# muzishen/RCDMs

Measured on AMD Instinct MI355X. Metric: story-frames/sec (stage-2 UNet, 50-step DDIM, 512^2), higher is better.
Workload: dtype f16; 1 GPU; PororoSV stage-2, 512x512, 50-step DDIM, CFG 2.0, batch=1 story x 5 frames per GPU, ctx 85x768, random-init 1276.9M-param UNet3D; stories_per_gpu=1, latent=64, ddim_steps=50, parallelism=story-replicas x1

## Files before the change

rcdms_amd/csrc/igemm16.hip:

```cpp
#include "common.h"
#include "igemm_args.h"
#include "pp_sync.h"
#include "igemm_epilogue.h"
#ifndef RCDM_I16_ABLATE
#define RCDM_I16_ABLATE 0
#endif

namespace {

template <int TAPS, bool SLAB>
__global__ __launch_bounds__(256, 2) void igemm16_kernel(const IgemmArgs p) {
  constexpr int BM = 160, BN = 160, FM = 5, FN = 5;
  constexpr int A_BYTES = BM * 128, STAGE = (BM + BN) * 128;
  constexpr int NP = BM / 8 / 4;
  extern __shared__ __attribute__((aligned(16))) char smem[];

  const int t = threadIdx.x, lane = t & 63;
  const int wave = __builtin_amdgcn_readfirstlane(t >> 6);
  const int wm = wave >> 1, wn = wave & 1;
  const int ks_begin = blockIdx.y * p.nk_per_split;
  const int nkl = min(p.nk, ks_begin + p.nk_per_split) - ks_begin;
  if (nkl <= 0) return;

  int cm0, cn0;
  {
    const int ntiles = p.tilesM * p.tilesN, lin = blockIdx.x;
    const int xcd = lin & 7, q = ntiles >> 3, r = ntiles & 7;
    const int tl = (xcd < r ? xcd * (q + 1) : r * (q + 1) + (xcd - r) * q) + (lin >> 3);
    constexpr int GM = 8;
    const int per_group = GM * p.tilesN;
    const int sg = tl / per_group, rem = tl - sg * per_group;
    const int gm = min(GM, p.tilesM - sg * GM);
    const int tn = rem / gm, tm = sg * GM + (rem - tn * gm);
    cm0 = tm * BM;
    cn0 = tn * BN;
  }

  f32x2 lx_pre = {1.f, 0.f};
  const bool lx_on = TAPS == 1 && !SLAB && p.lnx_stat != nullptr;
  LnxRow<1, kLnxMaxParts> lx_row0;
  if (lx_on && t < BM) lx_row0.load(p.lnx_stat, p.lnx_ld, cm0 + t, cm0 + t < p.M, p.lnx_parts, 0);

  const __amdgpu_buffer_rsrc_t rsrcA = __builtin_amdgcn_make_buffer_rsrc((void*)p.A, 0, 0x7FFFFFFF, 0x00020000);
  const __amdgpu_buffer_rsrc_t rsrcW = __builtin_amdgcn_make_buffer_rsrc((void*)p.W, 0, 0x7FFFFFFF, 0x00020000);
  const __amdgpu_buffer_rsrc_t rsrcA2 = __builtin_amdgcn_make_buffer_rsrc((void*)(TAPS == 9 ? p.A2 : p.A), 0, 0x7FFFFFFF, 0x00020000);
  constexpr unsigned OOB = 0x80000000u;
  const int Hv = p.Hi << p.up, Wv = p.Wi << p.up;
  const int lrow = lane >> 3, lch = lane & 7;

  unsigned a_off[NP], w_off[NP];
  int a_img[NP], a_iy[NP], a_ix[NP], a_c[NP], w_c[NP];
#pragma unroll
  for (int i = 0; i < NP; ++i) {
    const int row = (wave * NP + i) * 8 + lrow;
    const int m = cm0 + row;
    a_c[i] = (lch ^ ((row >> 1) & 7)) * 8;
    a_off[i] = OOB;
    a_img[i] = a_ix[i] = 0;
    a_iy[i] = -(1 << 20);
    if (TAPS == 1) {
      if (m < p.M) a_off[i] = (unsigned)m * (unsigned)p.lda * 2u;
    } else if (m < p.M) {
      const int hw = p.Ho * p.Wo;
      const int img = m / hw, rem = m - img * hw;
      const int oy = rem / p.Wo, ox = rem - oy * p.Wo;
      a_img[i] = img * p.Hi * p.Wi;
      a_iy[i] = oy * p.stride - p.pad;
      a_ix[i] = ox * p.stride - p.pad;
    }
    const int n = cn0 + row;
    w_c[i] = a_c[i];
    w_off[i] = n < p.N ? (unsigned)n * (unsigned)p.Ktot * 2u : OOB;
  }
  auto issue = [&](int g, int stage) __attribute__((always_inline)) {
    const int ks = ks_begin + g;
    int tap = 0, kci = ks;
    const bool s2 = TAPS == 9 && ks >= p.nk1;
    if (TAPS != 1) {
      kci = ks / 9;
      tap = ks - kci * 9;
      if (s2) {
        kci = ks - p.nk1;
        tap = 9;
      }
    }
    const int c0 = kci * BK;
    const int dy = s2 ? 1 : tap / 3, dx = s2 ? 1 : tap - dy * 3;
    const int cin = s2 ? p.Cin2 : p.Cin;
    const unsigned lda = (unsigned)(s2 ? p.lda2 : p.lda);
    char* sbase = smem + stage * STAGE;
#pragma unroll
    for (int i = 0; i < NP; ++i) {
      const int c = c0 + a_c[i];
      unsigned vo;
      if (TAPS == 1) {
        vo = (c < p.Cin && a_off[i] != OOB) ? a_off[i] + (unsigned)c * 2u : OOB;
      } else {
        const int iy = a_iy[i] + dy, ix = a_ix[i] + dx;
        const bool ok = (c < cin) && ((unsigned)iy < (unsigned)Hv) && ((unsigned)ix < (unsigned)Wv);
        const int sy = iy >> p.up, sx = ix >> p.up;
        const unsigned off = ((unsigned)(a_img[i] + sy * p.Wi + sx) * lda + (unsigned)c) * 2u;
        vo = ok ? off : OOB;
      }
      if (TAPS == 9 && s2)
        __builtin_amdgcn_raw_ptr_buffer_load_lds(
            rsrcA2, (__attribute__((address_space(3))) void*)(sbase + (wave * NP + i) * 1024), 16, vo, 0, 0, 0);
      else
        __builtin_amdgcn_raw_ptr_buffer_load_lds(
            rsrcA, (__attribute__((address_space(3))) void*)(sbase + (wave * NP + i) * 1024), 16, vo, 0, 0, 0);
    }
#if RCDM_I16_ABLATE & 16
    if (g > 0) return;
#endif
#pragma unroll
    for (int i = 0; i < NP; ++i) {
      const int c = c0 + w_c[i];
      const unsigned vo = (c < cin && w_off[i] != OOB)
                              ? w_off[i] + ((unsigned)tap * (unsigned)p.Cin + (unsigned)c) * 2u : OOB;
      __builtin_amdgcn_raw_ptr_buffer_load_lds(
          rsrcW, (__attribute__((address_space(3))) void*)(sbase + A_BYTES + (wave * NP + i) * 1024), 16, vo, 0, 0, 0);
    }
  };

  const int l15 = lane & 15, kg = lane >> 4;
  const int sw = (lane >> 1) & 7;
  const int koff0 = ((kg ^ sw) << 4), koff1 = (((4 + kg) ^ sw) << 4);
  const int rowA = (wm * (BM / 2) + l15) * 128, rowB = A_BYTES + (wn * (BN / 2) + l15) * 128;
  f32x4 acc[FN][FM];
#pragma unroll
  for (int i = 0; i < FN; ++i)
#pragma unroll
    for (int j = 0; j < FM; ++j) acc[i][j] = f32x4{0.f, 0.f, 0.f, 0.f};

  constexpr int kStg = BM * (2 * BN + 16);
  static_assert(lnx_table_bytes(BM, BN) <= 4096 && 4096 + kStg <= 2 * STAGE && kStg >= STAGE, "epilogue layout");
  const bool lx_low = lx_on && !(nkl & 1);
  float* const lx_tab = (float*)(smem + (lx_low ? 0 : kStg));
  char* const stg = smem + (lx_low ? 4096 : 0);
  issue(0, 0);
  if (lx_on && t < BM) {
    float r_ = 1.f, m_ = 0.f;
    lx_row0.finish(p.lnx_invC, p.lnx_eps, r_, m_);
    lx_pre = f32x2{r_, m_};
  }
  for (int g = 0; g < nkl; ++g) {
    wait_vm<0>();
    __builtin_amdgcn_s_barrier();
#if !(RCDM_I16_ABLATE & 8)
    if (g + 1 < nkl) issue(g + 1, (g + 1) & 1);
#endif
    const char* sb = smem + (g & 1) * STAGE;
#if RCDM_PRIO_LOADS
    __builtin_amdgcn_s_setprio(3);
#endif
#pragma unroll
    for (int kk = 0; kk < 2; ++kk) {
      const int koff = kk ? koff1 : koff0;
      f16x8 wf[FN], xf[FM];
#pragma unroll
      for (int i = 0; i < FN; ++i) wf[i] = *(const f16x8*)(sb + rowB + i * 2048 + koff);
#pragma unroll
      for (int j = 0; j < FM; ++j) xf[j] = *(const f16x8*)(sb + rowA + j * 2048 + koff);
#if RCDM_PRIO_LOADS
      __builtin_amdgcn_s_setprio(0);
#endif
#pragma unroll
      for (int i = 0; i < FN; ++i)
#pragma unroll
        for (int j = 0; j < FM; ++j) acc[i][j] = __builtin_amdgcn_mfma_f32_16x16x32_f16(wf[i], xf[j], acc[i][j], 0, 0, 0);
#if RCDM_PRIO_LOADS
      __builtin_amdgcn_s_setprio(3);
#endif
    }
  }
  if constexpr (TAPS == 1 && !SLAB)
    if (lx_on) lnx_write_tables<BM, BN>(p, lx_tab, cm0, cn0, t, lx_pre);
  wait_lgkm0();
  tick_barrier();
#if RCDM_I16_ABLATE & 1
  {
    float s = 0.f;
#pragma unroll
    for (int i = 0; i < FN; ++i)
#pragma unroll
      for (int j = 0; j < FM; ++j) s += acc[i][j][0] + acc[i][j][1] + acc[i][j][2] + acc[i][j][3];
    if (s == 1.2345678e33f) p.out[0] = (f16)s;
  }
#else
  if constexpr (SLAB) {
    if (p.slab16) {
      IgemmArgs q{};
      q.out = (f16*)p.partial + (size_t)blockIdx.y * p.M * p.N;
      q.M = p.M; q.N = p.N; q.ldc = p.N; q.epi = 0; q.out_scale = 1.0f; q.dup = 0;
      tile_epilogue<FM, FN, false, 256, BM, BN, false, false>(q, smem, acc, cm0, cn0, wm * (BM / 2), wn * (BN / 2), l15, kg, t, nullptr);
      return;
    }
  }
  tile_epilogue<FM, FN, SLAB, 256, BM, BN, false, TAPS == 1 && !SLAB>(p, stg, acc, cm0, cn0, wm * (BM / 2), wn * (BN / 2), l15, kg, t,
                                                                       lx_on ? lx_tab : nullptr);
#endif
}

constexpr int kLds16 = 2 * (160 + 160) * 128;

template <int TAPS>
int launch16(const IgemmArgs& a, hipStream_t stream) {
  static bool attr_set[64] = {};
  if (rcdm_first_on_device(attr_set)) {
    (void)hipFuncSetAttribute((const void*)igemm16_kernel<TAPS, false>, hipFuncAttributeMaxDynamicSharedMemorySize, kLds16);
    (void)hipFuncSetAttribute((const void*)igemm16_kernel<TAPS, true>, hipFuncAttributeMaxDynamicSharedMemorySize, kLds16);
  }
  dim3 grid(a.tilesM * a.tilesN, a.splits);
  if (a.splits > 1)
    hipLaunchKernelGGL((igemm16_kernel<TAPS, true>), grid, dim3(256), kLds16, stream, a);
  else
    hipLaunchKernelGGL((igemm16_kernel<TAPS, false>), grid, dim3(256), kLds16, stream, a);
  return rcdm_check_launch();
}

}

int rcdm_igemm16_launch(const IgemmArgs& a, int taps, hipStream_t stream) {
  if (taps == 1) return launch16<1>(a, stream);
  if (taps == 9) return launch16<9>(a, stream);
  return RCDM_EINVAL;
}
```

rcdms_amd/csrc/wino.hip:

```cpp
#include "common.h"
#include "igemm_args.h"
#include "pp_sync.h"
#include "igemm_epilogue.h"
#include <stdlib.h>

namespace {

struct WinoArgs {
  const f16* in;
  const f16* in2;
  const f16* U;
  const f16* W2;
  const float* bias;
  const float* rowvec;
  const f16* res;
  f16* out;
  f16* V;
  float* slab;
  int slab16;
  int n_img, H, W, th, tw, T, N, K, K2;
  int lda, lda2, ldc, ldr, ldt, rows_per_sample;
  int epi;
  float out_scale;
  int E, splits, nk, nk2, nkps, nkps2, tilesM, tilesN;
  const float* gn_stat;
  const float* gn_gamma;
  const float* gn_beta;
  int gn_cg, gn_G, gn_rps, gn_silu;
  float* go_partial;
  int go_G, go_cg, go_rps, go_splits;
};

__global__ __launch_bounds__(256) void wino_in_kernel(const WinoArgs p) {
  const int nch = p.K >> 2;
  const int idx = blockIdx.x * 256 + threadIdx.x;
  if (idx >= p.T * nch) return;
  const int t = idx / nch, c4 = idx - t * nch;
  const int tpi = p.th * p.tw;
  const int img = t / tpi, rem = t - img * tpi;
  const int ty = rem / p.tw, tx = rem - ty * p.tw;
  typedef unsigned u32x2_t __attribute__((ext_vector_type(2)));
  union H4 { u32x2_t v; f16 e[4]; f16x4 h; };
  const __amdgpu_buffer_rsrc_t rs = __builtin_amdgcn_make_buffer_rsrc((void*)p.in, 0, 0x7FFFFFFF, 0x00020000);
  const unsigned base = ((unsigned)(img * p.H * p.W) * (unsigned)p.lda + (unsigned)c4 * 4u) * 2u;
  H4 d[4][4];
  bool ok[4][4];
#pragma unroll
  for (int i = 0; i < 4; ++i)
#pragma unroll
    for (int j = 0; j < 4; ++j) {
      const int y = 2 * ty - 1 + i, x = 2 * tx - 1 + j;
      ok[i][j] = (unsigned)y < (unsigned)p.H && (unsigned)x < (unsigned)p.W;
      const unsigned off = ok[i][j] ? base + (unsigned)(y * p.W + x) * (unsigned)p.lda * 2u : 0x80000000u;
      d[i][j].v = __builtin_amdgcn_raw_buffer_load_b64(rs, off, 0, 0);
    }
  f32x4 sc = {1.f, 1.f, 1.f, 1.f}, sh = {0.f, 0.f, 0.f, 0.f};
  const bool gn = p.gn_stat != nullptr;
  if (gn) {
    const int s = (img * p.H * p.W) / p.gn_rps;
    const f32x4 ga = *(const f32x4*)(p.gn_gamma + c4 * 4), be = *(const f32x4*)(p.gn_beta + c4 * 4);
#pragma unroll
    for (int e = 0; e < 4; ++e) {
      const int g = (c4 * 4 + e) / p.gn_cg;
      const f32x2 mr = *(const f32x2*)(p.gn_stat + (size_t)(s * p.gn_G + g) * 2);
      sc[e] = mr.y * ga[e];
      sh[e] = __builtin_fmaf(-(mr.x * mr.y), ga[e], be[e]);
    }
  }
  float f[4][4][4];
#pragma unroll
  for (int i = 0; i < 4; ++i)
#pragma unroll
    for (int j = 0; j < 4; ++j)
#pragma unroll
      for (int e = 0; e < 4; ++e) {
        float v = (float)d[i][j].e[e];
        if (gn) {
          v = __builtin_fmaf(v, sc[e], sh[e]);
          if (p.gn_silu) v = silu_f(v);
          if (!ok[i][j]) v = 0.f;
        }
        f[i][j][e] = v;
      }
  float r[4][4][4];
#pragma unroll
  for (int j = 0; j < 4; ++j)
#pragma unroll
    for (int e = 0; e < 4; ++e) {
      r[0][j][e] = f[0][j][e] - f[2][j][e];
      r[1][j][e] = f[1][j][e] + f[2][j][e];
      r[2][j][e] = f[2][j][e] - f[1][j][e];
      r[3][j][e] = f[1][j][e] - f[3][j][e];
    }
  f16* vb = p.V + (size_t)t * p.K + c4 * 4;
  const size_t pstride = (size_t)p.T * p.K;
#pragma unroll
  for (int i = 0; i < 4; ++i) {
    H4 o[4];
#pragma unroll
    for (int e = 0; e < 4; ++e) {
      o[0].e[e] = (f16)(r[i][0][e] - r[i][2][e]);
      o[1].e[e] = (f16)(r[i][1][e] + r[i][2][e]);
      o[2].e[e] = (f16)(r[i][2][e] - r[i][1][e]);
      o[3].e[e] = (f16)(r[i][1][e] - r[i][3][e]);
    }
#pragma unroll
    for (int j = 0; j < 4; ++j) *(u32x2_t*)(vb + (size_t)(i * 4 + j) * pstride) = o[j].v;
  }
}

template <bool S16>
__global__ __launch_bounds__(256, 2) void wino_gemm_kernel(const WinoArgs p) {
  constexpr int BM = 160, BN = 160, FM = 5, FN = 5;
  constexpr int A_BYTES = BM * 128, STAGE = (BM + BN) * 128;
  constexpr int NP = BM / 8 / 4;
  extern __shared__ __attribute__((aligned(16))) char smem[];

  const int t = threadIdx.x, lane = t & 63;
  const int wave = __builtin_amdgcn_readfirstlane(t >> 6);
  const int wm = wave >> 1, wn = wave & 1;
  const int ntile = p.tilesM * p.tilesN, W = p.E * p.splits * ntile;
  const int n_extra = p.E - 16;
  int item;
  {
    const int lin = blockIdx.x, xcd = lin & 7, j = lin >> 3;
    const int WX = n_extra * p.splits * ntile, WM = W - WX;
    if (((WX | WM) & 7) == 0) {
      const int xq = WX >> 3, mq = WM >> 3;
      item = j < xq ? xcd * xq + j : WX + xcd * mq + (j - xq);
    } else {
      const int q = W >> 3, r = W & 7;
      item = (xcd < r ? xcd * (q + 1) : r * (q + 1) + (xcd - r) * q) + j;
    }
  }
  const int yes = item / ntile, tl = item - yes * ntile;
  const int ye = yes / p.splits, split = yes - ye * p.splits;
  const int entry = ye < n_extra ? 16 + ye : ye - n_extra;
  const bool extra = entry >= 16;
  const int nk = extra ? p.nk2 : p.nk, nkps = extra ? p.nkps2 : p.nkps;
  const int ks_begin = split * nkps;
  const int nkl = min(nk, ks_begin + nkps) - ks_begin;
  const int Kd = extra ? p.K2 : p.K;
  const size_t slab_off = ((size_t)entry * p.splits + split) * p.T * p.N;

  const int tn = tl / p.tilesM, tm = tl - tn * p.tilesM;
  const int cm0 = tm * BM, cn0 = tn * BN;
  const f16* Abase = extra ? p.in2 : p.V + (size_t)entry * p.T * p.K;
  const f16* Wbase = extra ? p.W2 : p.U + (size_t)entry * p.N * p.K;
  const __amdgpu_buffer_rsrc_t rsrcA = __builtin_amdgcn_make_buffer_rsrc((void*)Abase, 0, 0x7FFFFFFF, 0x00020000);
  const __amdgpu_buffer_rsrc_t rsrcW = __builtin_amdgcn_make_buffer_rsrc((void*)Wbase, 0, 0x7FFFFFFF, 0x00020000);
  constexpr unsigned OOB = 0x80000000u;
  const int lrow = lane >> 3, lch = lane & 7;

  unsigned a_off[NP], w_off[NP];
  int a_c[NP];
#pragma unroll
  for (int i = 0; i < NP; ++i) {
    const int row = (wave * NP + i) * 8 + lrow;
    const int m = cm0 + row;
    a_c[i] = (lch ^ ((row >> 1) & 7)) * 8;
    a_off[i] = OOB;
    if (m < p.T) {
      if (extra) {
        const int tpi = p.th * p.tw;
        const int img = m / tpi, rem = m - img * tpi;
        const int ty = rem / p.tw, tx = rem - ty * p.tw;
        const int ab = entry - 16;
        const int prow = img * p.H * p.W + (2 * ty + (ab >> 1)) * p.W + 2 * tx + (ab & 1);
        a_off[i] = (unsigned)prow * (unsigned)p.lda2 * 2u;
      } else {
        a_off[i] = (unsigned)m * (unsigned)p.K * 2u;
      }
    }
    const int n = cn0 + row;
    w_off[i] = n < p.N ? (unsigned)n * (unsigned)Kd * 2u : OOB;
  }
  auto issue = [&](int g, int stage) __attribute__((always_inline)) {
    const int c0 = (ks_begin + g) * BK;
    char* sbase = smem + stage * STAGE;
#pragma unroll
    for (int i = 0; i < NP; ++i) {
      const int c = c0 + a_c[i];
      const unsigned vo = (c < Kd && a_off[i] != OOB) ? a_off[i] + (unsigned)c * 2u : OOB;
      __builtin_amdgcn_raw_ptr_buffer_load_lds(
          rsrcA, (__attribute__((address_space(3))) void*)(sbase + (wave * NP + i) * 1024), 16, vo, 0, 0, 0);
    }
#pragma unroll
    for (int i = 0; i < NP; ++i) {
      const int c = c0 + a_c[i];
      const unsigned vo = (c < Kd && w_off[i] != OOB) ? w_off[i] + (unsigned)c * 2u : OOB;
      __builtin_amdgcn_raw_ptr_buffer_load_lds(
          rsrcW, (__attribute__((address_space(3))) void*)(sbase + A_BYTES + (wave * NP + i) * 1024), 16, vo, 0, 0, 0);
    }
  };

  const int l15 = lane & 15, kg = lane >> 4;
  const int sw = (lane >> 1) & 7;
  const int koff0 = ((kg ^ sw) << 4), koff1 = (((4 + kg) ^ sw) << 4);
  const int rowA = (wm * (BM / 2) + l15) * 128, rowB = A_BYTES + (wn * (BN / 2) + l15) * 128;
  f32x4 acc[FN][FM];
#pragma unroll
  for (int i = 0; i < FN; ++i)
#pragma unroll
    for (int j = 0; j < FM; ++j) acc[i][j] = f32x4{0.f, 0.f, 0.f, 0.f};

  if (nkl > 0) issue(0, 0);
  for (int g = 0; g < nkl; ++g) {
    wait_vm<0>();
    __builtin_amdgcn_s_barrier();
    if (g + 1 < nkl) issue(g + 1, (g + 1) & 1);
    const char* sb = smem + (g & 1) * STAGE;
    __builtin_amdgcn_s_setprio(3);
#pragma unroll
    for (int kk = 0; kk < 2; ++kk) {
      const int koff = kk ? koff1 : koff0;
      f16x8 wf[FN], xf[FM];
#pragma unroll
      for (int i = 0; i < FN; ++i) wf[i] = *(const f16x8*)(sb + rowB + i * 2048 + koff);
#pragma unroll
      for (int j = 0; j < FM; ++j) xf[j] = *(const f16x8*)(sb + rowA + j * 2048 + koff);
      __builtin_amdgcn_s_setprio(0);
#pragma unroll
      for (int i = 0; i < FN; ++i)
#pragma unroll
        for (int j = 0; j < FM; ++j) acc[i][j] = __builtin_amdgcn_mfma_f32_16x16x32_f16(wf[i], xf[j], acc[i][j], 0, 0, 0);
      __builtin_amdgcn_s_setprio(3);
    }
  }
  const int row0 = wm * (BM / 2), col0 = wn * (BN / 2);
  if constexpr (S16) {
    wait_lgkm0();
    tick_barrier();
    IgemmArgs q{};
    q.out = (f16*)p.slab + slab_off;
    q.M = p.T; q.N = p.N; q.ldc = p.N; q.epi = 0; q.out_scale = 1.0f; q.dup = 0;
    tile_epilogue<FM, FN, false, 256, BM, BN, false, false>(q, smem, acc, cm0, cn0, row0, col0, l15, kg, t, nullptr);
  } else {
    wait_lgkm0();
    tick_barrier();
    slab_store_staged<FM, FN, 256, BM, BN, 80>(p.slab + slab_off, p.N, p.T, p.N, smem, acc, cm0, cn0, row0, col0, l15, kg, t);
  }
}

template <bool S16>
__device__ __forceinline__ f32x4 slab_load4(const WinoArgs& p, size_t off) {
  if constexpr (S16) {
    union { uint2 u; f16 e[4]; } h;
    h.u = *(const uint2*)((const f16*)p.slab + off);
    return f32x4{(float)h.e[0], (float)h.e[1], (float)h.e[2], (float)h.e[3]};
  } else {
    return *(const f32x4*)(p.slab + off);
  }
}

template <int SP, bool S16>
__global__ __launch_bounds__(512) void wino_out_kernel(const WinoArgs p) {
  extern __shared__ __attribute__((aligned(16))) char smem[];
  const int nch = p.N >> 2;
  const int t = blockIdx.x;
  const int tpi = p.th * p.tw;
  const int img = t / tpi, rem = t - img * tpi;
  const int ty = rem / p.tw, tx = rem - ty * p.tw;
  const size_t splane = (size_t)p.T * p.N, eplane = (size_t)p.splits * splane;
  int prow[4];
#pragma unroll
  for (int ab = 0; ab < 4; ++ab) prow[ab] = img * p.H * p.W + (2 * ty + (ab >> 1)) * p.W + 2 * tx + (ab & 1);
  union H4 { uint2 u; f16 e[4]; };
  for (int cg4 = threadIdx.x; cg4 < nch; cg4 += blockDim.x) {
    const int n = cg4 * 4;
    const size_t src = (size_t)t * p.N + n;
    H4 rr[4];
#pragma unroll
    for (int ab = 0; ab < 4; ++ab) {
      rr[ab].u = make_uint2(0, 0);
      if (p.epi & RCDM_EPI_RESIDUAL) rr[ab].u = *(const uint2*)(p.res + (size_t)prow[ab] * p.ldr + n);
    }
    f32x4 m[16];
#pragma unroll
    for (int e = 0; e < 16; ++e) m[e] = slab_load4<S16>(p, src + e * eplane);
    if constexpr (SP == 2) {
      f32x4 m2[16];
#pragma unroll
      for (int e = 0; e < 16; ++e) m2[e] = slab_load4<S16>(p, src + e * eplane + splane);
#pragma unroll
      for (int e = 0; e < 16; ++e) m[e] += m2[e];
    } else if constexpr (SP == 0) {
      for (int s = 1; s < p.splits; ++s) {
        f32x4 m2[16];
#pragma unroll
        for (int e = 0; e < 16; ++e) m2[e] = slab_load4<S16>(p, src + e * eplane + s * splane);
#pragma unroll
        for (int e = 0; e < 16; ++e) m[e] += m2[e];
      }
    }
    f32x4 o[4];
    {
      f32x4 r0[4], r1[4];
#pragma unroll
      for (int j = 0; j < 4; ++j) {
        r0[j] = m[0 * 4 + j] + m[1 * 4 + j] + m[2 * 4 + j];
        r1[j] = m[1 * 4 + j] - m[2 * 4 + j] - m[3 * 4 + j];
      }
      o[0] = r0[0] + r0[1] + r0[2];
      o[1] = r0[1] - r0[2] - r0[3];
      o[2] = r1[0] + r1[1] + r1[2];
      o[3] = r1[1] - r1[2] - r1[3];
    }
    if (p.E > 16) {
      f32x4 x[4];
#pragma unroll
      for (int ab = 0; ab < 4; ++ab) x[ab] = slab_load4<S16>(p, src + (16 + ab) * eplane);
      for (int s = 1; s < p.splits; ++s) {
#pragma unroll
        for (int ab = 0; ab < 4; ++ab) x[ab] += slab_load4<S16>(p, src + (16 + ab) * eplane + s * splane);
      }
#pragma unroll
      for (int ab = 0; ab < 4; ++ab) o[ab] += x[ab];
    }
    f32x4 add = {0.f, 0.f, 0.f, 0.f};
    if (p.epi & RCDM_EPI_BIAS) add += *(const f32x4*)(p.bias + n);
    if (p.epi & RCDM_EPI_ROWVEC) add += *(const f32x4*)(p.rowvec + (size_t)(prow[0] / p.rows_per_sample) * p.ldt + n);
    f32x4 cs = {0.f, 0.f, 0.f, 0.f}, cq = cs;
#pragma unroll
    for (int ab = 0; ab < 4; ++ab) {
      H4 q;
#pragma unroll
      for (int e = 0; e < 4; ++e) {
        q.e[e] = (f16)((o[ab][e] + add[e] + (float)rr[ab].e[e]) * p.out_scale);
        const float f = (float)q.e[e];
        cs[e] += f;
        cq[e] += f * f;
      }
      *(uint2*)(p.out + (size_t)prow[ab] * p.ldc + n) = q.u;
    }
    if (p.go_partial) {
      *(f32x4*)(smem + (size_t)n * 4) = cs;
      *(f32x4*)(smem + (size_t)(p.N + n) * 4) = cq;
    }
  }
  if (p.go_partial) {
    __syncthreads();
    const int g = threadIdx.x;
    if (g < p.go_G) {
      const float* fs = (const float*)smem;
      float gs = 0.f, gq = 0.f;
      for (int c = g * p.go_cg; c < (g + 1) * p.go_cg; ++c) {
        gs += fs[c];
        gq += fs[p.N + c];
      }
      const float nn = 4.f * (float)p.go_cg;
      const float mean = gs / nn;
      float m2 = gq - gs * mean;
      if (m2 < 0.f) m2 = 0.f;
      const int s = prow[0] / p.go_rps;
      const int sp = t - s * p.go_splits;
      float* o = p.go_partial + (((size_t)s * p.go_G + g) * p.go_splits + sp) * 3;
      o[0] = nn;
      o[1] = mean;
      o[2] = m2;
    }
  }
}

__global__ __launch_bounds__(256) void wino_pack_kernel(const float* __restrict__ w, f16* __restrict__ U, int c_out, int c_in) {
  const size_t idx = (size_t)blockIdx.x * 256 + threadIdx.x;
  const size_t total = (size_t)c_out * c_in;
  if (idx >= total) return;
  const float* g = w + idx * 9;
  float gg[3][3];
#pragma unroll
  for (int i = 0; i < 3; ++i)
#pragma unroll
    for (int j = 0; j < 3; ++j) gg[i][j] = g[i * 3 + j];
  float r[4][3];
#pragma unroll
  for (int j = 0; j < 3; ++j) {
    r[0][j] = gg[0][j];
    r[1][j] = 0.5f * (gg[0][j] + gg[1][j] + gg[2][j]);
    r[2][j] = 0.5f * (gg[0][j] - gg[1][j] + gg[2][j]);
    r[3][j] = gg[2][j];
  }
#pragma unroll
  for (int i = 0; i < 4; ++i) {
    const float u0 = r[i][0], u1 = 0.5f * (r[i][0] + r[i][1] + r[i][2]), u2 = 0.5f * (r[i][0] - r[i][1] + r[i][2]), u3 = r[i][2];
    U[(size_t)(i * 4 + 0) * total + idx] = (f16)u0;
    U[(size_t)(i * 4 + 1) * total + idx] = (f16)u1;
    U[(size_t)(i * 4 + 2) * total + idx] = (f16)u2;
    U[(size_t)(i * 4 + 3) * total + idx] = (f16)u3;
  }
}

struct UpGatherArgs {
  const f16* P;
  const float* bias;
  f16* out;
  int ldp, ldc, n_img, H, W, C;
  int up;
};
__global__ __launch_bounds__(256) void upsample_gather_kernel(const UpGatherArgs p) {
  const int nch = p.C >> 3;
  const size_t total = ((size_t)p.n_img * p.H * p.W << (2 * p.up)) * nch;
  const size_t idx = (size_t)blockIdx.x * 256 + threadIdx.x;
  if (idx >= total) return;
  const int o = (int)(idx / nch), c8 = (int)(idx - (size_t)o * nch);
  const int W2 = p.W << p.up, H2 = p.H << p.up;
  const int img = o / (H2 * W2), rem = o - img * (H2 * W2);
  const int Y = rem / W2, X = rem - Y * W2;
  const __amdgpu_buffer_rsrc_t rs = __builtin_amdgcn_make_buffer_rsrc((void*)p.P, 0, 0x7FFFFFFF, 0x00020000);
  Pack16 v[9];
#pragma unroll
  for (int ky = 0; ky < 3; ++ky)
#pragma unroll
    for (int kx = 0; kx < 3; ++kx) {
      const int yy = Y + ky - 1, xx = X + kx - 1;
      const bool ok = (unsigned)yy < (unsigned)H2 && (unsigned)xx < (unsigned)W2;
      const unsigned row = (unsigned)(img * p.H * p.W + (yy >> p.up) * p.W + (xx >> p.up));
      const unsigned off = ok ? (row * (unsigned)p.ldp + (unsigned)((ky * 3 + kx) * p.C + c8 * 8)) * 2u : 0x80000000u;
      v[ky * 3 + kx].v = __builtin_amdgcn_raw_buffer_load_b128(rs, off, 0, 0);
    }
  float acc[8];
#pragma unroll
  for (int e = 0; e < 8; ++e) acc[e] = 0.f;
  if (p.bias) {
    const f32x4 b0 = *(const f32x4*)(p.bias + c8 * 8), b1 = *(const f32x4*)(p.bias + c8 * 8 + 4);
#pragma unroll
    for (int e = 0; e < 4; ++e) {
      acc[e] = b0[e];
      acc[4 + e] = b1[e];
    }
  }
#pragma unroll
  for (int k = 0; k < 9; ++k)
#pragma unroll
    for (int e = 0; e < 8; ++e) acc[e] += (float)v[k].e[e];
  Pack16 q;
#pragma unroll
  for (int e = 0; e < 8; ++e) q.e[e] = (f16)acc[e];
  *(uint4*)(p.out + (size_t)o * p.ldc + c8 * 8) = q.u;
}

int g_wino_cus = 0;
int wino_cus() {
  if (g_wino_cus <= 0) {
    int dev = 0, n = 0;
    if (hipGetDevice(&dev) == hipSuccess && hipDeviceGetAttribute(&n, hipDeviceAttributeMultiprocessorCount, dev) == hipSuccess && n > 0)
      g_wino_cus = n;
    else
      g_wino_cus = 256;
  }
  return g_wino_cus;
}

inline size_t align256(size_t v) { return (v + 255) & ~(size_t)255; }

int wino_plan(const rcdm_conv3x3_desc* d, WinoArgs& a) {
  if (!d) return RCDM_EINVAL;
  if (d->n_img <= 0 || d->h_in <= 0 || d->w_in <= 0 || d->c_in <= 0 || d->c_out <= 0) return RCDM_EINVAL;
  if (d->stride != 1 || d->upsample != 0 || d->pad_after_only || d->dup_rows) return RCDM_ESHAPE;
  if ((d->h_in & 1) || (d->w_in & 1)) return RCDM_ESHAPE;
  if ((d->c_in & 63) || (d->c_out & 7) || (d->c_in2 & 63)) return RCDM_ESHAPE;
  if ((d->lda & 7) || (d->ldc & 7) || (d->c_in2 && (d->lda2 & 7))) return RCDM_EINVAL;
  if (d->epilogue & ~(RCDM_EPI_BIAS | RCDM_EPI_ROWVEC | RCDM_EPI_RESIDUAL)) return RCDM_ESHAPE;
  if ((d->epilogue & RCDM_EPI_RESIDUAL) && (d->ldr & 7)) return RCDM_EINVAL;
  a = WinoArgs{};
  a.n_img = d->n_img; a.H = d->h_in; a.W = d->w_in;
  a.th = d->h_in / 2; a.tw = d->w_in / 2;
  a.T = d->n_img * a.th * a.tw;
  a.N = d->c_out; a.K = d->c_in; a.K2 = d->c_in2;
  a.lda = d->lda; a.lda2 = d->lda2; a.ldc = d->ldc; a.ldr = d->ldr; a.ldt = d->ldt;
  a.rows_per_sample = d->rows_per_sample > 0 ? d->rows_per_sample : 1;
  a.epi = d->epilogue;
  a.out_scale = d->out_scale == 0.f ? 1.f : d->out_scale;
  a.E = d->c_in2 ? 20 : 16;
  a.nk = d->c_in / BK; a.nk2 = d->c_in2 / BK;
  a.tilesM = (a.T + 159) / 160; a.tilesN = (a.N + 159) / 160;
  if ((size_t)a.T * a.K * 2 >= (1ull << 31)) return RCDM_ESHAPE;
  if ((size_t)d->n_img * d->h_in * d->w_in * d->lda * 2 >= (1ull << 31)) return RCDM_ESHAPE;
  if (d->c_in2 && (size_t)d->n_img * d->h_in * d->w_in * d->lda2 * 2 >= (1ull << 31)) return RCDM_ESHAPE;
  if ((size_t)a.N * (a.K > a.K2 ? a.K : a.K2) * 2 >= (1ull << 31)) return RCDM_ESHAPE;
  int splits = d->split_k;
  if (splits <= 0) {
    const int blocks = a.E * a.tilesM * a.tilesN;
    splits = wino_cus() / (blocks > 0 ? blocks : 1);
    if (splits > a.nk / 5) splits = a.nk / 5;
    if (splits > 8) splits = 8;
  }
  if (splits < 1) splits = 1;
  if (splits > a.nk) splits = a.nk;
  a.splits = splits;
  a.nkps = (a.nk + splits - 1) / splits;
  a.nkps2 = (a.nk2 + splits - 1) / splits;
  return RCDM_OK;
}
size_t wino_v_bytes(const WinoArgs& a) { return align256((size_t)16 * a.T * a.K * 2); }
size_t wino_slab_bytes(const WinoArgs& a) { return align256((size_t)a.E * a.splits * a.T * a.N * 4); }

int g_wino_slab16 = -1;
int wino_slab16() {
  if (g_wino_slab16 < 0) {
    const char* e = getenv("RCDM_WINO_SLAB16");
    g_wino_slab16 = e ? (atoi(e) != 0) : 1;
  }
  return g_wino_slab16;
}

}

extern "C" {

int rcdm_conv3x3_wino_supported(const rcdm_conv3x3_desc* d) {
  WinoArgs a;
  return wino_plan(d, a) == RCDM_OK ? 1 : 0;
}

size_t rcdm_conv3x3_wino_workspace_bytes(const rcdm_conv3x3_desc* d) {
  WinoArgs a;
  if (wino_plan(d, a) != RCDM_OK) return 0;
  return wino_v_bytes(a) + wino_slab_bytes(a);
}

int rcdm_conv3x3_wino_plan_query(const rcdm_conv3x3_desc* d, int32_t* out8) {
  WinoArgs a;
  const int rc = wino_plan(d, a);
  if (rc != RCDM_OK || !out8) return rc != RCDM_OK ? rc : RCDM_EINVAL;
  out8[0] = 11; out8[1] = 160; out8[2] = 160; out8[3] = a.tilesM; out8[4] = a.tilesN * a.E; out8[5] = a.splits; out8[6] = 2;
  out8[7] = a.nk;
  return RCDM_OK;
}

int rcdm_conv_taps_gather(const void* P, int32_t ldp, int32_t n_img, int32_t h, int32_t w, int32_t c_out, int32_t upsample,
                          const float* bias, void* out, int32_t ldc, void* stream) {
  if (!P || !out || n_img <= 0 || h <= 0 || w <= 0 || c_out <= 0 || (upsample != 0 && upsample != 1)) return RCDM_EINVAL;
  if ((c_out & 7) || (ldp & 7) || (ldc & 7) || ldp < 9 * c_out || ldc < c_out) return RCDM_EINVAL;
  if ((((uintptr_t)P | (uintptr_t)out | (uintptr_t)bias) & 15)) return RCDM_EINVAL;
  if ((size_t)n_img * h * w * ldp * 2 >= (1ull << 31)) return RCDM_ESHAPE;
  UpGatherArgs a{(const f16*)P, bias, (f16*)out, ldp, ldc, n_img, h, w, c_out, upsample};
  const size_t total = ((size_t)n_img * h * w << (2 * upsample)) * (c_out >> 3);
  hipLaunchKernelGGL(upsample_gather_kernel, dim3((unsigned)((total + 255) / 256)), dim3(256), 0, (hipStream_t)stream, a);
  return rcdm_check_launch();
}

int rcdm_upsample_taps_gather(const void* P, int32_t ldp, int32_t n_img, int32_t h, int32_t w, int32_t c_out, const float* bias,
                              void* out, int32_t ldc, void* stream) {
  return rcdm_conv_taps_gather(P, ldp, n_img, h, w, c_out, 1, bias, out, ldc, stream);
}

int rcdm_set_wino_slab_f16(int32_t on) {
  g_wino_slab16 = on < 0 ? -1 : (on ? 1 : 0);
  return RCDM_OK;
}

int rcdm_pack_conv3x3_wino(const float* w, int32_t c_out, int32_t c_in, void* dst, void* stream) {
  if (!w || !dst || c_out <= 0 || c_in <= 0) return RCDM_EINVAL;
  const size_t total = (size_t)c_out * c_in;
  hipLaunchKernelGGL(wino_pack_kernel, dim3((unsigned)((total + 255) / 256)), dim3(256), 0, (hipStream_t)stream, w, (f16*)dst, c_out, c_in);
  return rcdm_check_launch();
}

int rcdm_conv3x3_wino(const rcdm_conv3x3_desc* d, const rcdm_groupnorm_desc* gn, const float* gn_stat, const float* gn_gamma,
                      const float* gn_beta, const void* in, const void* in2, const void* U, const void* W2, const float* bias,
                      const float* rowvec, const void* residual, void* out, void* workspace, size_t workspace_bytes,
                      const rcdm_groupnorm_desc* gn_out, float* gn_out_partial, void* stream_) {
  WinoArgs a;
  const int rc = wino_plan(d, a);
  if (rc != RCDM_OK) return rc;
  if (!in || !U || !out || !workspace) return RCDM_EINVAL;
  if ((d->c_in2 != 0) != (in2 != nullptr) || (d->c_in2 != 0) != (W2 != nullptr)) return RCDM_EINVAL;
  if ((a.epi & RCDM_EPI_BIAS) && !bias) return RCDM_EINVAL;
  if ((a.epi & RCDM_EPI_ROWVEC) && (!rowvec || (d->ldt & 3))) return RCDM_EINVAL;
  if ((a.epi & RCDM_EPI_RESIDUAL) && !residual) return RCDM_EINVAL;
  if (workspace_bytes < wino_v_bytes(a) + wino_slab_bytes(a)) return RCDM_EWORKSPACE;
  if (((uintptr_t)in | (uintptr_t)out | (uintptr_t)U | (uintptr_t)workspace | (uintptr_t)in2 | (uintptr_t)W2 | (uintptr_t)residual |
       (uintptr_t)bias | (uintptr_t)rowvec) & 15)
    return RCDM_EINVAL;
  if (gn) {
    if (!gn_stat || !gn_gamma || !gn_beta) return RCDM_EINVAL;
    if (gn->C != d->c_in || gn->groups <= 0 || gn->C % gn->groups || gn->samples * gn->rows_per_sample != d->n_img * d->h_in * d->w_in ||
        gn->rows_per_sample % (d->h_in * d->w_in))
      return RCDM_ESHAPE;
    a.gn_stat = gn_stat; a.gn_gamma = gn_gamma; a.gn_beta = gn_beta;
    a.gn_G = gn->groups; a.gn_cg = gn->C / gn->groups; a.gn_rps = gn->rows_per_sample; a.gn_silu = gn->silu;
  }
  if (gn_out) {
    if (!gn_out_partial) return RCDM_EINVAL;
    if (gn_out->C != d->c_out || gn_out->groups <= 0 || gn_out->groups > 64 || gn_out->C % gn_out->groups ||
        gn_out->samples * gn_out->rows_per_sample != d->n_img * d->h_in * d->w_in || gn_out->rows_per_sample % (d->h_in * d->w_in) ||
        a.N * 8 > 64 * 1024)
      return RCDM_ESHAPE;
    a.go_partial = gn_out_partial;
    a.go_G = gn_out->groups; a.go_cg = gn_out->C / gn_out->groups; a.go_rps = gn_out->rows_per_sample;
    a.go_splits = gn_out->rows_per_sample / 4;
  }
  a.in = (const f16*)in; a.in2 = (const f16*)in2; a.U = (const f16*)U; a.W2 = (const f16*)W2;
  a.bias = bias; a.rowvec = rowvec; a.res = (const f16*)residual; a.out = (f16*)out;
  a.V = (f16*)workspace;
  a.slab16 = wino_slab16();
  a.slab = (float*)((char*)workspace + wino_v_bytes(a));
  hipStream_t stream = (hipStream_t)stream_;
  {
    const size_t items = (size_t)a.T * (a.K >> 2);
    hipLaunchKernelGGL(wino_in_kernel, dim3((unsigned)((items + 255) / 256)), dim3(256), 0, stream, a);
  }
  {
    constexpr int kLds = 2 * (160 + 160) * 128;
    static bool attr_set[64] = {};
    if (rcdm_first_on_device(attr_set)) {
      (void)hipFuncSetAttribute((const void*)wino_gemm_kernel<false>, hipFuncAttributeMaxDynamicSharedMemorySize, kLds);
      (void)hipFuncSetAttribute((const void*)wino_gemm_kernel<true>, hipFuncAttributeMaxDynamicSharedMemorySize, kLds);
    }
    if (a.slab16) hipLaunchKernelGGL(wino_gemm_kernel<true>, dim3(a.tilesM * a.tilesN * a.E * a.splits), dim3(256), kLds, stream, a);
    else hipLaunchKernelGGL(wino_gemm_kernel<false>, dim3(a.tilesM * a.tilesN * a.E * a.splits), dim3(256), kLds, stream, a);
  }
  {
    int threads = ((a.N >> 2) + 63) / 64 * 64;
    if (threads > 512) threads = 512;
    const size_t lds = a.go_partial ? (size_t)a.N * 8 : 0;
    const dim3 grid((unsigned)a.T);
    if (a.slab16) {
      if (a.splits == 1) hipLaunchKernelGGL((wino_out_kernel<1, true>), grid, dim3(threads), lds, stream, a);
      else if (a.splits == 2) hipLaunchKernelGGL((wino_out_kernel<2, true>), grid, dim3(threads), lds, stream, a);
      else hipLaunchKernelGGL((wino_out_kernel<0, true>), grid, dim3(threads), lds, stream, a);
    } else {
      if (a.splits == 1) hipLaunchKernelGGL((wino_out_kernel<1, false>), grid, dim3(threads), lds, stream, a);
      else if (a.splits == 2) hipLaunchKernelGGL((wino_out_kernel<2, false>), grid, dim3(threads), lds, stream, a);
      else hipLaunchKernelGGL((wino_out_kernel<0, false>), grid, dim3(threads), lds, stream, a);
    }
  }
  return rcdm_check_launch();
}

}
```

Before: 5.982 story-frames/s.

## Software-pipeline igemm16 and Winograd k-loops, interleaving LDS reads and DMA with MFMAs

Replaces the simple double-buffered k-loop in the 160x160 igemm16 and Winograd GEMM kernels with a shared, hand-scheduled loop. The fragments for the next k-half are prefetched from LDS while the current MFMAs run. The global-to-LDS buffer loads are split into per-row pieces and interleaved one per MFMA slot, with sched_barrier pinning the order. The goal is to hide LDS read latency and load-issue cost behind matrix math and to cut the once-per-step barrier stall. In exchange it adds register pressure from two fragment sets and a fixed instruction schedule that the compiler can no longer reorder.

Result: no change. 5.965 story-frames/s (median of 2 runs) (-0.3%).

```diff
diff --git a/rcdms_amd/csrc/i16_loop.h b/rcdms_amd/csrc/i16_loop.h
--- /dev/null
+++ b/rcdms_amd/csrc/i16_loop.h
@@ -0,0 +1,107 @@
+#pragma once
+#include "common.h"
+#include "igemm_args.h"
+#include "pp_sync.h"
+
+namespace i16 {
+
+constexpr int kBM = 160, kBN = 160, kFM = 5, kFN = 5;
+constexpr int kABytes = kBM * 128, kStage = (kBM + kBN) * 128;
+constexpr int kNP = kBM / 8 / 4;
+constexpr int kPieces = 2 * kNP;
+
+struct Frags {
+  f16x8 w[kFN], x[kFM];
+};
+
+__device__ __forceinline__ void read_frag(Frags& f, int r, const char* sb, int rowA, int rowB, int koff) {
+  if (r < kFN) f.w[r] = *(const f16x8*)(sb + rowB + r * 2048 + koff);
+  else f.x[r - kFN] = *(const f16x8*)(sb + rowA + (r - kFN) * 2048 + koff);
+}
+
+__device__ __forceinline__ void read_frags(Frags& f, const char* sb, int rowA, int rowB, int koff) {
+#pragma unroll
+  for (int r = 0; r < kFN + kFM; ++r) read_frag(f, r, sb, rowA, rowB, koff);
+}
+
+__device__ __forceinline__ void mfma_k(f32x4 (&acc)[kFN][kFM], const Frags& f, int k) {
+  const int i = k / kFM, j = k % kFM;
+  acc[i][j] = __builtin_amdgcn_mfma_f32_16x16x32_f16(f.w[i], f.x[j], acc[i][j], 0, 0, 0);
+}
+
+__device__ __forceinline__ void mfma_half(f32x4 (&acc)[kFN][kFM], const Frags& f) {
+#pragma unroll
+  for (int k = 0; k < kFN * kFM; ++k) mfma_k(acc, f, k);
+}
+
+template <bool DMA, class Piece>
+__device__ __forceinline__ void cluster(f32x4 (&acc)[kFN][kFM], const Frags& use, Frags& next, const char* nsb, int rowA,
+                                        int rowB, int koff, const Piece& piece) {
+  constexpr int kSlots = kFN + kFM;
+  static_assert(!DMA || kPieces == kSlots, "one piece per slot");
+  __builtin_amdgcn_sched_barrier(0);
+  int k = 0;
+#pragma unroll
+  for (int r = 0; r < kSlots; ++r) {
+    mfma_k(acc, use, k++);
+    __builtin_amdgcn_sched_barrier(0);
+    if constexpr (DMA) {
+      piece(r);
+      __builtin_amdgcn_sched_barrier(0);
+      mfma_k(acc, use, k++);
+      __builtin_amdgcn_sched_barrier(0);
+    }
+    read_frag(next, r, nsb, rowA, rowB, koff);
+    __builtin_amdgcn_sched_barrier(0);
+  }
+#pragma unroll
+  for (; k < kFN * kFM; ++k) mfma_k(acc, use, k);
+  __builtin_amdgcn_sched_barrier(0);
+}
+
+__device__ __forceinline__ void step_barrier() {
+  __builtin_amdgcn_sched_barrier(0);
+  __builtin_amdgcn_s_waitcnt(0x0070);
+  __builtin_amdgcn_s_barrier();
+  __builtin_amdgcn_sched_barrier(0);
+}
+
+template <class Issue>
+__device__ __forceinline__ void kloop(f32x4 (&acc)[kFN][kFM], const char* smem, int nkl, int rowA, int rowB, int koff0,
+                                      int koff1, const Issue& issue) {
+  const auto none = [](int) {};
+  Frags f0, f1;
+  step_barrier();
+  read_frags(f0, smem, rowA, rowB, koff0);
+  if (nkl > 1) {
+#pragma unroll
+    for (int p = 0; p < kPieces; ++p) issue(1, 1, p);
+  }
+  __builtin_amdgcn_s_waitcnt(0xC07F);
+  int g = 0;
+  for (; g + 2 < nkl; ++g) {
+    cluster<false>(acc, f0, f1, smem + (g & 1) * kStage, rowA, rowB, koff1, none);
+    step_barrier();
+#if RCDM_PRIO_LOADS
+    __builtin_amdgcn_s_setprio(3);
+#endif
+    cluster<true>(acc, f1, f0, smem + ((g + 1) & 1) * kStage, rowA, rowB, koff0,
+                  [&](int p) { issue(g + 2, g & 1, p); });
+#if RCDM_PRIO_LOADS
+    __builtin_amdgcn_s_setprio(0);
+#endif
+  }
+  if (g + 1 < nkl) {
+    cluster<false>(acc, f0, f1, smem + (g & 1) * kStage, rowA, rowB, koff1, none);
+    step_barrier();
+    cluster<false>(acc, f1, f0, smem + ((g + 1) & 1) * kStage, rowA, rowB, koff0, none);
+    ++g;
+  }
+  cluster<false>(acc, f0, f1, smem + (g & 1) * kStage, rowA, rowB, koff1, none);
+  mfma_half(acc, f1);
+#if RCDM_PRIO_LOADS
+  __builtin_amdgcn_s_setprio(3);
+#endif
+}
+
+}
diff --git a/rcdms_amd/csrc/igemm16.hip b/rcdms_amd/csrc/igemm16.hip
--- a/rcdms_amd/csrc/igemm16.hip
+++ b/rcdms_amd/csrc/igemm16.hip
@@ -2,6 +2,7 @@
 #include "igemm_args.h"
 #include "pp_sync.h"
 #include "igemm_epilogue.h"
+#include "i16_loop.h"
 #ifndef RCDM_I16_ABLATE
 #define RCDM_I16_ABLATE 0
 #endif
@@ -13,6 +14,7 @@
   constexpr int BM = 160, BN = 160, FM = 5, FN = 5;
   constexpr int A_BYTES = BM * 128, STAGE = (BM + BN) * 128;
   constexpr int NP = BM / 8 / 4;
+  static_assert(BM == i16::kBM && BN == i16::kBN && A_BYTES == i16::kABytes && STAGE == i16::kStage && NP == i16::kNP, "i16_loop.h tile");
   extern __shared__ __attribute__((aligned(16))) char smem[];
 
   const int t = threadIdx.x, lane = t & 63;
@@ -72,7 +74,7 @@
     w_c[i] = a_c[i];
     w_off[i] = n < p.N ? (unsigned)n * (unsigned)p.Ktot * 2u : OOB;
   }
-  auto issue = [&](int g, int stage) __attribute__((always_inline)) {
+  auto issue = [&](int g, int stage, int q) __attribute__((always_inline)) {
     const int ks = ks_begin + g;
     int tap = 0, kci = ks;
     const bool s2 = TAPS == 9 && ks >= p.nk1;
@@ -89,8 +91,11 @@
     const int cin = s2 ? p.Cin2 : p.Cin;
     const unsigned lda = (unsigned)(s2 ? p.lda2 : p.lda);
     char* sbase = smem + stage * STAGE;
-#pragma unroll
-    for (int i = 0; i < NP; ++i) {
+#if RCDM_I16_ABLATE & 8
+    if (g > 0) return;
+#endif
+    if (q < NP) {
+      const int i = q;
       const int c = c0 + a_c[i];
       unsigned vo;
       if (TAPS == 1) {
@@ -108,12 +113,11 @@
       else
         __builtin_amdgcn_raw_ptr_buffer_load_lds(
             rsrcA, (__attribute__((address_space(3))) void*)(sbase + (wave * NP + i) * 1024), 16, vo, 0, 0, 0);
-    }
+    } else {
 #if RCDM_I16_ABLATE & 16
-    if (g > 0) return;
-#endif
-#pragma unroll
-    for (int i = 0; i < NP; ++i) {
+      if (g > 0) return;
+#endif
+      const int i = q - NP;
       const int c = c0 + w_c[i];
       const unsigned vo = (c < cin && w_off[i] != OOB)
                               ? w_off[i] + ((unsigned)tap * (unsigned)p.Cin + (unsigned)c) * 2u : OOB;
@@ -137,42 +141,14 @@
   const bool lx_low = lx_on && !(nkl & 1);
   float* const lx_tab = (float*)(smem + (lx_low ? 0 : kStg));
   char* const stg = smem + (lx_low ? 4096 : 0);
-  issue(0, 0);
+#pragma unroll
+  for (int q = 0; q < i16::kPieces; ++q) issue(0, 0, q);
   if (lx_on && t < BM) {
     float r_ = 1.f, m_ = 0.f;
     lx_row0.finish(p.lnx_invC, p.lnx_eps, r_, m_);
     lx_pre = f32x2{r_, m_};
   }
-  for (int g = 0; g < nkl; ++g) {
-    wait_vm<0>();
-    __builtin_amdgcn_s_barrier();
-#if !(RCDM_I16_ABLATE & 8)
-    if (g + 1 < nkl) issue(g + 1, (g + 1) & 1);
-#endif
-    const char* sb = smem + (g & 1) * STAGE;
-#if RCDM_PRIO_LOADS
-    __builtin_amdgcn_s_setprio(3);
-#endif
-#pragma unroll
-    for (int kk = 0; kk < 2; ++kk) {
-      const int koff = kk ? koff1 : koff0;
-      f16x8 wf[FN], xf[FM];
-#pragma unroll
-      for (int i = 0; i < FN; ++i) wf[i] = *(const f16x8*)(sb + rowB + i * 2048 + koff);
-#pragma unroll
-      for (int j = 0; j < FM; ++j) xf[j] = *(const f16x8*)(sb + rowA + j * 2048 + koff);
-#if RCDM_PRIO_LOADS
-      __builtin_amdgcn_s_setprio(0);
-#endif
-#pragma unroll
-      for (int i = 0; i < FN; ++i)
-#pragma unroll
-        for (int j = 0; j < FM; ++j) acc[i][j] = __builtin_amdgcn_mfma_f32_16x16x32_f16(wf[i], xf[j], acc[i][j], 0, 0, 0);
-#if RCDM_PRIO_LOADS
-      __builtin_amdgcn_s_setprio(3);
-#endif
-    }
-  }
+  i16::kloop(acc, smem, nkl, rowA, rowB, koff0, koff1, issue);
   if constexpr (TAPS == 1 && !SLAB)
     if (lx_on) lnx_write_tables<BM, BN>(p, lx_tab, cm0, cn0, t, lx_pre);
   wait_lgkm0();
diff --git a/rcdms_amd/csrc/wino.hip b/rcdms_amd/csrc/wino.hip
--- a/rcdms_amd/csrc/wino.hip
+++ b/rcdms_amd/csrc/wino.hip
@@ -2,6 +2,7 @@
 #include "igemm_args.h"
 #include "pp_sync.h"
 #include "igemm_epilogue.h"
+#include "i16_loop.h"
 #include <stdlib.h>
 
 namespace {
@@ -114,6 +115,7 @@
   constexpr int BM = 160, BN = 160, FM = 5, FN = 5;
   constexpr int A_BYTES = BM * 128, STAGE = (BM + BN) * 128;
   constexpr int NP = BM / 8 / 4;
+  static_assert(BM == i16::kBM && BN == i16::kBN && A_BYTES == i16::kABytes && STAGE == i16::kStage && NP == i16::kNP, "i16_loop.h tile");
   extern __shared__ __attribute__((aligned(16))) char smem[];
 
   const int t = threadIdx.x, lane = t & 63;
@@ -175,18 +177,16 @@
     const int n = cn0 + row;
     w_off[i] = n < p.N ? (unsigned)n * (unsigned)Kd * 2u : OOB;
   }
-  auto issue = [&](int g, int stage) __attribute__((always_inline)) {
+  auto issue = [&](int g, int stage, int q) __attribute__((always_inline)) {
     const int c0 = (ks_begin + g) * BK;
     char* sbase = smem + stage * STAGE;
-#pragma unroll
-    for (int i = 0; i < NP; ++i) {
-      const int c = c0 + a_c[i];
-      const unsigned vo = (c < Kd && a_off[i] != OOB) ? a_off[i] + (unsigned)c * 2u : OOB;
+    if (q < NP) {
+      const int c = c0 + a_c[q];
+      const unsigned vo = (c < Kd && a_off[q] != OOB) ? a_off[q] + (unsigned)c * 2u : OOB;
       __builtin_amdgcn_raw_ptr_buffer_load_lds(
-          rsrcA, (__attribute__((address_space(3))) void*)(sbase + (wave * NP + i) * 1024), 16, vo, 0, 0, 0);
-    }
-#pragma unroll
-    for (int i = 0; i < NP; ++i) {
+          rsrcA, (__attribute__((address_space(3))) void*)(sbase + (wave * NP + q) * 1024), 16, vo, 0, 0, 0);
+    } else {
+      const int i = q - NP;
       const int c = c0 + a_c[i];
       const unsigned vo = (c < Kd && w_off[i] != OOB) ? w_off[i] + (unsigned)c * 2u : OOB;
       __builtin_amdgcn_raw_ptr_buffer_load_lds(
@@ -204,28 +204,10 @@
 #pragma unroll
     for (int j = 0; j < FM; ++j) acc[i][j] = f32x4{0.f, 0.f, 0.f, 0.f};
 
-  if (nkl > 0) issue(0, 0);
-  for (int g = 0; g < nkl; ++g) {
-    wait_vm<0>();
-    __builtin_amdgcn_s_barrier();
-    if (g + 1 < nkl) issue(g + 1, (g + 1) & 1);
-    const char* sb = smem + (g & 1) * STAGE;
-    __builtin_amdgcn_s_setprio(3);
-#pragma unroll
-    for (int kk = 0; kk < 2; ++kk) {
-      const int koff = kk ? koff1 : koff0;
-      f16x8 wf[FN], xf[FM];
-#pragma unroll
-      for (int i = 0; i < FN; ++i) wf[i] = *(const f16x8*)(sb + rowB + i * 2048 + koff);
-#pragma unroll
-      for (int j = 0; j < FM; ++j) xf[j] = *(const f16x8*)(sb + rowA + j * 2048 + koff);
-      __builtin_amdgcn_s_setprio(0);
-#pragma unroll
-      for (int i = 0; i < FN; ++i)
-#pragma unroll
-        for (int j = 0; j < FM; ++j) acc[i][j] = __builtin_amdgcn_mfma_f32_16x16x32_f16(wf[i], xf[j], acc[i][j], 0, 0, 0);
-      __builtin_amdgcn_s_setprio(3);
-    }
+  if (nkl > 0) {
+#pragma unroll
+    for (int q = 0; q < i16::kPieces; ++q) issue(0, 0, q);
+    i16::kloop(acc, smem, nkl, rowA, rowB, koff0, koff1, issue);
   }
   const int row0 = wm * (BM / 2), col0 = wn * (BN / 2);
   if constexpr (S16) {
```
